# Hanbo-Cheng/DAWN-pytorch

Hardware: AMD Instinct MI355X
Metric: generated frames/sec at 256x256, 50 DDIM steps (higher is better)
Workload: dtype f32

## Files before the change

dawn-pytorch_amd/_lib.py:

```python
from __future__ import annotations

import ctypes as C
import os
from pathlib import Path

_HERE = Path(__file__).resolve().parent
LIB_PATH = Path(os.environ.get("DAWN_HIP_LIB", str(_HERE / "libdawn_hip.so")))

c_f = C.c_void_p
_i, _l, _f, _d = C.c_int, C.c_long, C.c_float, C.c_double


class ConvDesc(C.Structure):
    _fields_ = [
        ("in0", c_f), ("in1", c_f),
        ("C0", _i), ("C1", _i), ("ld0", _i), ("ld1", _i),
        ("F", _i), ("Hi", _i), ("Wi", _i), ("Ho", _i), ("Wo", _i),
        ("KH", _i), ("KW", _i), ("stride", _i), ("pad", _i),
        ("mode", _i),
        ("w", c_f), ("bias", c_f),
        ("N", _i),
        ("row_mean", c_f), ("row_rstd", c_f),
        ("ch_a", c_f), ("ch_b", c_f),
        ("pro_act", _i),
# ... 31 lines not shown
    "dawn_gn_finalize": [c_f, _d, c_f, c_f, c_f, c_f, _i, _f, c_f, c_f, c_f],
    "dawn_gn_reduce_finalize": [c_f, _i, _d, c_f, c_f, c_f, c_f, _i, _f, c_f, c_f, c_f],
    "dawn_gn_ticket_reset": [c_f, c_f],
    "dawn_gn_apply_res": [c_f, c_f, c_f, c_f, c_f, _l, _i, c_f],
    "dawn_ln_rowstats": [c_f, _i, _i, c_f, _i, _i, _l, _f, c_f, c_f, c_f],
    "dawn_ln_rows": [c_f, _i, _i, c_f, _i, _i, _l, _f, c_f, c_f],
    "dawn_xattn_prep": [c_f, _i, c_f, c_f, c_f, _i, c_f, c_f],
    "dawn_xattn_core": [c_f, c_f, _l, _i, c_f, c_f, c_f, c_f],
    "dawn_xattn_ln_sum": [c_f, c_f, c_f, _l, _i, _f, c_f],
    "dawn_xattn_tables": [c_f, c_f, c_f, c_f, c_f, c_f, _i, _i, c_f, c_f],
    "dawn_xattn_sigma_out": [c_f, _l, _i, c_f, c_f, _i, _f, c_f, c_f],
    "dawn_xattn_sigma_out_h1": [c_f, _l, _i, c_f, c_f, _i, _f, c_f, c_f, c_f, c_f, c_f],
    "dawn_xattn_layer_c64": [c_f, _i, _i, c_f, _i, _i, _l, _i, c_f, c_f, c_f, c_f, _f, c_f, c_f],
    "dawn_xattn_layer_c64_h1": [c_f, _i, _i, c_f, _i, _i, _l, _i, c_f, c_f, c_f, c_f, _f, c_f, c_f, c_f, c_f, c_f],
    "dawn_temporal_attn": [c_f, _i, _i, _i, _i, _i, c_f, c_f, c_f, c_f, c_f],
    "dawn_temporal_attn_ex": [c_f, _i, _i, _i, _i, _i, c_f, c_f, c_f, c_f, _i, c_f],
    "dawn_temporal_layer_c64": [c_f, _i, _i, _i, _i, _i, c_f, c_f, c_f, c_f, c_f, c_f, _f, c_f, c_f],
    "dawn_temporal_layer_c64_ex": [c_f, _i, _i, _i, _i, _i, c_f, c_f, c_f, c_f, c_f, c_f, c_f, _f, c_f, _i, c_f],
    "dawn_tl16_schedule": [_i, _i, _i, _i, c_f, c_f],
    "dawn_tl13_schedule": [_i, _i, _i, _i, c_f],
    "dawn_sla_context": [c_f, _i, _i, c_f, c_f],
    "dawn_sla_apply": [c_f, c_f, _i, _i, c_f, c_f],
    "dawn_sla_ws_floats": [_i, _i, _i],
    "dawn_gemm1x1_split_ok": [_l, _i, _i, _i],
    "dawn_gemm1x1_ln_inline_ok": [_l, _i, _i, _i],
    "dawn_sla_layer_c64": [c_f, _i, _i, c_f, c_f, c_f, c_f, _f, c_f, c_f, c_f],
    "dawn_frame_attn": [c_f, _i, _i, c_f, c_f],
    "dawn_init_conv_x": [c_f, c_f, c_f, _i, _i, _i, _i, c_f, c_f],
    "dawn_init_conv_x_ex": [c_f, _l, c_f, c_f, _i, _i, _i, _i, c_f, c_f],
    "dawn_head_out": [c_f, c_f, c_f, c_f, c_f, c_f, _l, _i, c_f, c_f],
    "dawn_heads_eps": [c_f, c_f, c_f, c_f, c_f, c_f, c_f, _i, _i, c_f, _i, _i, c_f, c_f, c_f, c_f, _l, _i, c_f, c_f],
    "dawn_fold_heads": [c_f, c_f, c_f, c_f, c_f, c_f, c_f, c_f, _i, _i, c_f, c_f],
    "dawn_linear": [c_f, _i, _i, _i, c_f, c_f, _i, _i, c_f, _i, c_f],
    "dawn_sinusoidal": [_f, _i, c_f, c_f, c_f],
    "dawn_ddim_x0": [c_f, c_f, _f, _f, _l, c_f, c_f, c_f],
    "dawn_select_scan": [c_f, _i, C.c_ulonglong, c_f, _i, c_f],
    "dawn_select_hist": [c_f, _l, c_f, _i, c_f, c_f],
    "dawn_select_finalize": [c_f, c_f, _f, c_f, c_f],
    "dawn_select_ws_reset": [c_f, c_f],
    "dawn_attn_bias32": [c_f, _i, c_f, _i, c_f, _i, _i, _i, _i, c_f, c_f, c_f, _i, _f, c_f, _i, c_f],
    "dawn_attn_win32": [c_f, _i, c_f, _i, c_f, _i, _i, _i, _i, _i, c_f, c_f, c_f, _i, _f, c_f, _i, c_f],
    "dawn_ubench_mfma_bf16": [_i, _i, c_f, c_f, C.POINTER(C.c_float), c_f],
    "dawn_ddim_update": [c_f, c_f, c_f, c_f, _f, _f, _f, _l, c_f, c_f],
    "dawn_cfg_combine": [c_f, c_f, _f, _l, c_f, c_f],
    "dawn_cfg_x0": [c_f, c_f, _f, c_f, _f, _f, _l, c_f, c_f, c_f, c_f],
    "dawn_workspace_bytes_guided": [c_f, _i, _i, _i, _i, _i],
# ... 97 lines not shown
CTX_SIGNATURES = {
    "dawn_ctx_create": [c_f, c_f, _i, c_f],
    "dawn_ctx_destroy": [c_f],
    "dawn_ctx_set_option": [c_f, _i, _i],
    "dawn_clip_bytes": [c_f, _i, _i, _i],
    "dawn_workspace_bytes": [c_f, _i, _i, _i],
    "dawn_workspace_bytes_sharded": [c_f, _i, _i, _i, _i, _i],
    "dawn_clip_prepare": [c_f, _i, _i, _i, c_f, c_f, _i, c_f, c_f, c_f, C.c_size_t, c_f, C.c_size_t, c_f],
    "dawn_unet_forward": _fwd + [c_f],
    "dawn_unet_forward_sharded": _fwd + [c_f, c_f],
    "dawn_sampler_run": _run + [c_f],
    "dawn_sampler_run_sharded": _run + [c_f, c_f],
    "dawn_ctx_profile_read": [c_f, c_f, _i],
    "dawn_rel_pos_bucket": [_i],
}

_lib = None


class DawnHipError(RuntimeError):
    pass


LONG_RESULT = {"dawn_sla_ws_floats", "dawn_workspace_bytes_guided", "dawn_decoder_skip_bytes", "dawn_decoder_workspace_bytes",
               "dawn_hubert_conv_frames", "dawn_hubert_workspace_bytes", "dawn_pbnet_workspace_bytes",
               "dawn_pose_blink_workspace_bytes", "dawn_clip_bytes", "dawn_workspace_bytes",
               "dawn_workspace_bytes_sharded", "dawn_image_ingest_workspace_bytes", "dawn_resample16k_len",
               "dawn_resample16k_workspace_bytes", "dawn_bundle_device_bytes",
               "dawn_bundle_verify_workspace_bytes"}


def lib() -> C.CDLL:
    global _lib
    if _lib is None:
        if not LIB_PATH.exists():
            raise DawnHipError(
                f"{LIB_PATH} not found: the HIP extension is mandatory (no CPU fallback). "
                "Build it with `python -c 'import __graft_entry__ as g; g.build()'` or ./build_lib.sh")
        L = C.CDLL(str(LIB_PATH))
        L.dawn_last_error.restype = C.c_char_p
        L.dawn_abi_version.restype = _i
        for name, args in {**SIGNATURES, **CTX_HELPER_SIGNATURES, **CTX_SIGNATURES}.items():
            fn = getattr(L, name)
            fn.argtypes = args
            fn.restype = _l if name in LONG_RESULT else _i
        _lib = L
    return _lib
# ... 6 lines not shown
```

dawn-pytorch_amd/csrc/dawn_ctx.hip:

```cpp
#include "dawn_host.h"

#include <math.h>
#include <string.h>
#include <iterator>
#include <vector>

extern "C" int dawn_gemm1x1_split_ok(long M, int N, int C0, int C1);
extern "C" int dawn_gemm1x1_ln_inline_ok(long M, int N, int C0, int C1);

namespace {

#define HCK(expr)                                                     \
    do {                                                              \
        const hipError_t e__ = (expr);                                \
        if (e__ != hipSuccess) return dawn_set_error(e__, __FILE__, __LINE__); \
    } while (0)

struct RB {
    int Cin = 0, Co = 0;
    bool conditioned = false;
    int cond_index = -1, film_off = 0;
    const float *w1 = nullptr, *b1 = nullptr, *g1 = nullptr, *be1 = nullptr, *w2 = nullptr, *b2 = nullptr, *g2 = nullptr,
                *be2 = nullptr, *wr = nullptr, *br = nullptr;
    const void *w1s = nullptr, *w2s = nullptr, *wrs = nullptr, *wqs = nullptr, *w1w = nullptr, *w2w = nullptr, *w1w4 = nullptr, *w2w4 = nullptr;
// ... 19 lines not shown
struct ProfEntry { hipEvent_t e0, e1; double flops, bytes; int kind; };

}

struct dawn_ctx {
    dawn_unet_cfg cfg;
    int dims[10];
    const float *w3, *wfea, *b_init, *sin_freqs, *t_w1, *t_b1, *t_w2, *t_b2, *film_w, *film_b, *wg, *bg, *wo, *bo;
    AT init_tattn;
    std::vector<Level> downs, ups;
    RB mid1, mid2, head_g, head_o;
    AT mid_sattn, mid_tattn;
    int n_cond = 0, film_total = 0, time_dim = 0;
    float rel_emb[32 * 8];
    float rot_freqs[16];
    const float* rot_freqs_dev = nullptr;
    std::vector<float> host_tab;
    hipStream_t side = nullptr;
    hipEvent_t ev_fork = nullptr, ev_join = nullptr;
    int conv_policy = 0, temporal_flags = 0, overlap = 1;
    int up_border = 0;
    int long_clip_frames = 4096;
    int fold_heads = 1;
    float* heads_fold = nullptr;
    Arena arena;
    bool prof_on = false;
    std::vector<ProfEntry> prof;
    std::vector<hipEvent_t> ev_pool;
};

namespace {

void load_rb(dawn_ctx* c, DawnWeights& Wt, const std::string& p, int Cin, int Co, bool conditioned, RB& rb, int& film_off) {
    auto F = [&](const std::string& n) { return Wt.getf(p + n); };
    auto V = [&](const std::string& n) { return Wt.opt(p + n); };
    rb.Cin = Cin; rb.Co = Co; rb.conditioned = conditioned;
    rb.w1 = F("w1"); rb.b1 = F("b1"); rb.g1 = F("g1"); rb.be1 = F("be1");
    rb.w2 = F("w2"); rb.b2 = F("b2"); rb.g2 = F("g2"); rb.be2 = F("be2");
    rb.w1s = V("w1s"); rb.w2s = V("w2s"); rb.w1w = V("w1w"); rb.w2w = V("w2w"); rb.w1w4 = V("w1w4"); rb.w2w4 = V("w2w4");
    if (Cin != Co) { rb.wr = F("wr"); rb.br = F("br"); rb.wrs = V("wrs"); }
    if (conditioned) {
        rb.cond_index = c->n_cond++;
        rb.film_off = film_off;
        film_off += 2 * Co;
        rb.wq = F("wq"); rb.wqs = V("wqs"); rb.q_scale = F("q_scale"); rb.g3 = F("g3");
        for (int b = 0; b < 3; ++b) {
// ... 491 lines not shown
    }
    T2 spatial_linear(const AT& a, const T2& x, int Fr, int H, int W, bool inplace = false) {
        const int HW = H * W;
        T2 o;
        if (a.C == 64) {
            float* ws = falloc((size_t)dawn_sla_ws_floats(Fr, HW, a.wqkv_s != nullptr));
            o = inplace ? x : t2(x.rows, 64);
            LAUNCH(dawn_sla_layer_c64(x.p, Fr, HW, a.wqkv, a.wqkv_s, a.wout, a.bout, 1e-5f, ws, o.p, cur));
            A.free(ws);
            return o;
        }
        return per_frame_attention(a, x, Fr, H, W, true);
    }
    T2 mid_spatial(const AT& a, const T2& x, int Fr, int H, int W) { return per_frame_attention(a, x, Fr, H, W, false); }
    T2 per_frame_attention(const AT& a, const T2& x, int Fr, int H, int W, bool linear) {
        const int HW = H * W;
        T2 o = t2(x.rows, a.C);
        const int step = Fr > c->long_clip_frames ? 256 : Fr;
        for (int fa = 0; fa < Fr; fa += step) {
            const int fb = fa + step < Fr ? fa + step : Fr, Fc = fb - fa;
            T2 xv;
            xv.p = x.p + (size_t)fa * HW * a.C; xv.rows = (long)Fc * HW; xv.C = a.C;
            T2 qkv = ln_gemm(xv, nullptr, a.wqkv, 768, a.wqkv_s, Fc, H, W);
            T2 at = t2(xv.rows, 256);
            if (linear) {
                float* ctx = falloc((size_t)Fc * 8 * 32 * 32);
                LAUNCH(dawn_sla_context(qkv.p, Fc, HW, ctx, cur));
                LAUNCH(dawn_sla_apply(qkv.p, ctx, Fc, HW, at.p, cur));
                A.free(ctx);
            } else {
                LAUNCH(dawn_frame_attn(qkv.p, Fc, HW, at.p, cur));
            }
            rel(qkv);
            ConvArgs g;
            g.in0 = at.p; g.C0 = 256; g.ld0 = 256; g.w = a.wout; g.w_bf3 = a.wout_s; g.bias = linear ? a.bout : nullptr; g.N = a.C;
            g.Fr = Fc; g.Hi = H; g.Wi = W; g.res = xv.p; g.ld_res = a.C; g.out = o.p + (size_t)fa * HW * a.C; g.ld_out = a.C;
            conv(g);
            rel(at);
        }
        return o;
    }

    void forward(const float* x3, float t, float* eps_out) {
        float* film = begin(t);
        T2 r, x;
        init_layers(x3, r, x);
// ... 266 lines not shown
    if (c->ev_join) (void)hipEventDestroy(c->ev_join);
    for (auto& p : c->prof) { (void)hipEventDestroy(p.e0); (void)hipEventDestroy(p.e1); }
    for (auto e : c->ev_pool) (void)hipEventDestroy(e);
    if (c->heads_fold) (void)hipFree(c->heads_fold);
    delete c;
}

extern "C" int dawn_ctx_set_option(dawn_ctx* c, int option, int value) {
    if (option == DAWN_OPT_UP_BORDER && (value < 0 || value > 2))
        return dawn_set_error_msg(-204, "dawn_ctx_set_option: DAWN_OPT_UP_BORDER is 0 (zero), 1 (edge) or 2 (wrap)");
    if (!c) return dawn_set_error_msg(-202, "dawn_ctx_set_option: null ctx");
    switch (option) {
        case DAWN_OPT_CONV_POLICY: c->conv_policy = value; return 0;
        case DAWN_OPT_TEMPORAL_FLAGS: c->temporal_flags = value; return 0;
        case DAWN_OPT_OVERLAP: c->overlap = value ? 1 : 0; return 0;
        case DAWN_OPT_LONG_CLIP_FRAMES: c->long_clip_frames = value > 0 ? value : 4096; return 0;
        case DAWN_OPT_UP_BORDER: c->up_border = value; return 0;
        case DAWN_OPT_FOLD_HEADS: c->fold_heads = value ? 1 : 0; return 0;
        case DAWN_OPT_PROFILE:
            c->prof_on = value != 0;
            return 0;
        default: return dawn_set_error_msg(-204, "dawn_ctx_set_option: unknown option");
    }
}

extern "C" size_t dawn_clip_bytes(dawn_ctx* c, int F, int h, int w) {
    if (!c || F <= 0 || h <= 0 || w <= 0) return 0;
    return clip_layout(c, F, h, w).total;
}

static size_t clip_scratch_bytes(dawn_ctx* c, int F, int h, int w) {
    int maxCo = 0;
    for (int l = 0; l <= c->cfg.n_levels; ++l) maxCo = c->dims[l] > maxCo ? c->dims[l] : maxCo;
    return al256((size_t)h * w * c->cfg.fea_ch * 4) + al256((size_t)F * 2 * maxCo * 4) + al256((size_t)F * 128 * 4) + 4096;
}

extern "C" int dawn_clip_prepare(dawn_ctx* c, int F, int h, int w, const float* fea272, const float* cond, int ld_cond,
                                 const float* rot_cos, const float* rot_sin, void* clip_mem, size_t clip_bytes,
                                 void* workspace, size_t workspace_bytes, void* stream) {
    if (!c || !fea272 || !cond || !clip_mem) return dawn_set_error_msg(-202, "dawn_clip_prepare: null argument");
    const ClipLayout L = clip_layout(c, F, h, w);
    if (clip_bytes < L.total) return dawn_set_error_msg(-205, "dawn_clip_prepare: clip memory too small (dawn_clip_bytes)");
    if (workspace_bytes < clip_scratch_bytes(c, F, h, w)) return dawn_set_error_msg(-201, "dawn_clip_prepare: workspace too small");
    hipStream_t s = (hipStream_t)stream;
    char* cm = (char*)clip_mem;
    char* ws = (char*)workspace;
// ... 335 lines not shown
```

dawn-pytorch_amd/csrc/spatial_attn.hip:

```cpp
#include "dawn_common.h"
#include "../../include/dawn_hip.h"

namespace {

constexpr int HEADS = 8, DH = 32, QKV = 768;

__global__ __launch_bounds__(512) void sla_context_kernel(const float* __restrict__ qkv, int HW,
                                                          float* __restrict__ ctx) {
    __shared__ float dens[HEADS * DH];
    const int f = blockIdx.x;
    const int tid = threadIdx.x;
    const int h = tid >> 6, lane = tid & 63;
    const int l31 = lane & 31, half = lane >> 5;
    const float* base = qkv + (long)f * HW * QKV + h * DH + l31;
    constexpr float LOG2E = 1.4426950408889634f;
    float kn[16], vn[16];
    auto request = [&](int t0) __attribute__((always_inline)) {
#pragma unroll
        for (int s = 0; s < 16; ++s) {
            const int n = t0 + 16 * half + s;
            const bool ok = n < HW;
            const float* r = base + (long)(ok ? n : HW - 1) * QKV;
            kn[s] = ok ? r[HEADS * DH] : -3.0e38f;
            vn[s] = ok ? r[2 * HEADS * DH] : 0.f;
// ... 79 lines not shown
            for (int c = 0; c < 4; ++c)
#pragma unroll
                for (int e = 0; e < 4; ++e) {
                    q4[c][e] = __builtin_amdgcn_exp2f((q4[c][e] - mx) * 1.4426950408889634f);
                    sm += q4[c][e];
                }
            sm += __shfl_xor(sm, 32, 64);
            const float inv = 0.17677669529663687f / sm;
            f32x16 acc;
#pragma unroll
            for (int r = 0; r < 16; ++r) acc[r] = 0.f;
#pragma unroll
            for (int c = 0; c < 4; ++c) {
                const f32x4 a4 = *reinterpret_cast<const f32x4*>(cT + (h * DH + l31) * 36 + 16 * half + 4 * c);
#pragma unroll
                for (int e = 0; e < 4; ++e) acc = __builtin_amdgcn_mfma_f32_32x32x2f32(a4[e], q4[c][e] * inv, acc, 0, 0, 0);
            }
            if (ok) {
#pragma unroll
                for (int g = 0; g < 4; ++g)
                    *reinterpret_cast<f32x4*>(orow + h * DH + 8 * g + 4 * half) =
                        f32x4{acc[4 * g], acc[4 * g + 1], acc[4 * g + 2], acc[4 * g + 3]};
            }
        }
    }
}

__global__ __launch_bounds__(64) void frame_attn_kernel(const float* __restrict__ qkv, int N,
                                                        float* __restrict__ out) {
    extern __shared__ __attribute__((aligned(16))) float kv[];
    float* ks = kv;
    float* vs = kv + (long)N * DH;
    const int f = blockIdx.x / HEADS, h = blockIdx.x % HEADS;
    const int lane = threadIdx.x;
    const float* base = qkv + (long)f * N * QKV + h * DH;
    for (int i = lane; i < N * DH; i += 64) {
        const int n = i >> 5, c = i & 31;
        ks[i] = base[(long)n * QKV + HEADS * DH + c];
        vs[i] = base[(long)n * QKV + 2 * HEADS * DH + c];
    }
    __syncthreads();
    for (int i0 = 0; i0 < N; i0 += 64) {
        const int i = i0 + lane;
        const bool ok = i < N;
        float q[DH], o[DH];
#pragma unroll
// ... 23 lines not shown
#pragma unroll
            for (int d = 0; d < DH; d += 4) {
                f32x4 v = {o[d] * inv, o[d + 1] * inv, o[d + 2] * inv, o[d + 3] * inv};
                *reinterpret_cast<f32x4*>(op + d) = v;
            }
        }
    }
}

}

extern "C" int dawn_sla_context(const float* qkv, int F, int HW, float* ctx, void* stream) {
    hipLaunchKernelGGL(sla_context_kernel, dim3(F), dim3(512), 0, (hipStream_t)stream, qkv, HW, ctx);
    DAWN_LAUNCH_CHECK();
    return 0;
}
extern "C" int dawn_sla_apply(const float* qkv, const float* ctx, int F, int HW, float* out, void* stream) {
    const int rpb = 512;
    hipLaunchKernelGGL(sla_apply_kernel, dim3(dawn_cdiv(HW, rpb), F), dim3(256), 0, (hipStream_t)stream, qkv, ctx, HW,
                       rpb, out);
    DAWN_LAUNCH_CHECK();
    return 0;
}
extern "C" int dawn_frame_attn(const float* qkv, int F, int N, float* out, void* stream) {
    if (N > 256) return dawn_set_error_msg(-40, "dawn_frame_attn: more than 256 tokens per frame not supported");
    const size_t lds = (size_t)N * DH * 2 * sizeof(float);
    hipLaunchKernelGGL(frame_attn_kernel, dim3(F * HEADS), dim3(64), lds, (hipStream_t)stream, qkv, N, out);
    DAWN_LAUNCH_CHECK();
    return 0;
}
```

dawn-pytorch_amd/ctx.py:

```python
from __future__ import annotations

import ctypes as C
import os
from typing import Dict, List, Optional, Sequence

import torch

from . import _lib
from ._lib import check
from .pack import PackedAttn, PackedResBlock, PackedUNet

Tensor = torch.Tensor


class UnetCfg(C.Structure):
    _fields_ = [("dim", C.c_int), ("n_levels", C.c_int), ("dim_mults", C.c_int * 8), ("fea_ch", C.c_int),
                ("cond_aud", C.c_int), ("cond_pose", C.c_int), ("cond_eye", C.c_int), ("win", C.c_int)]


class NamedPtr(C.Structure):
    _fields_ = [("name", C.c_char_p), ("ptr", C.c_void_p)]


class DdimStep(C.Structure):
# ... 169 lines not shown
            self._ws = None
            self._ws = torch.empty(nbytes, dtype=torch.uint8, device=self.device)
        return self._ws


class CtxEvaluator(_Evaluator):

    def __init__(self, P: PackedUNet):
        self.P = P
        cfg = UnetCfg()
        cfg.dim, cfg.n_levels = P.dim, P.n_levels
        for i in range(P.n_levels):
            cfg.dim_mults[i] = P.dims[i + 1] // P.dim
        cfg.fea_ch = P.fea_ch
        cfg.cond_aud, cfg.cond_pose, cfg.cond_eye = P.cond_dims
        cfg.win = P.win
        super().__init__("dawn_ctx_create", "dawn_ctx_destroy", cfg, named_weights(P), P.rel_emb.device, fp32_only=False)
        self._need = {}
        self._policy = 0
        if P.up_border:
            self.set_option(OPT_UP_BORDER, P.up_border)
        if os.environ.get("DAWN_FOLD_HEADS", "1") == "0":
            self.set_option(OPT_FOLD_HEADS, 0)

    def set_option(self, option: int, value: int) -> None:
        check(self.L.dawn_ctx_set_option(self.h, option, int(value)), "dawn_ctx_set_option")
        if option == OPT_CONV_POLICY:
            self._policy = int(value)
        if option != OPT_PROFILE:
            self._need.clear()

    def workspace(self, F: int, h: int, w: int, shard: Optional[ShardCallbacks] = None, guided: bool = False) -> Tensor:
        key = (F, h, w, self._policy, None if shard is None else (shard.rank, shard.world))
        if guided:
            key = key + ("guided",)
        need = self._need.get(key)
        if need is None:
            if guided:
                rank, world = (0, 1) if shard is None else (shard.rank, shard.world)
                need = self._need[key] = int(self.L.dawn_workspace_bytes_guided(self.h, F, h, w, rank, world))
            else:
                need = self._need[key] = int(self.L.dawn_workspace_bytes(self.h, F, h, w) if shard is None else
                                             self.L.dawn_workspace_bytes_sharded(self.h, F, h, w, shard.rank, shard.world))
        return self._grown(need)

    def prepare_clip(self, fea272: Tensor, cond: Tensor, rcos: Optional[Tensor] = None, rsin: Optional[Tensor] = None) -> dict:
        Cf, h, w = fea272.shape
        F = cond.shape[0]
        if not (fea272.is_cuda and fea272.is_contiguous() and cond.is_cuda and cond.stride(1) == 1 and fea272.dtype == torch.float32
                and cond.dtype == torch.float32):
            raise _lib.DawnHipError("prepare_clip: fea272 must be a contiguous fp32 GPU tensor, cond an fp32 GPU tensor with unit column stride")
        mem = torch.empty(int(self.L.dawn_clip_bytes(self.h, F, h, w)), dtype=torch.uint8, device=self.device)
        ws = self.workspace(F, h, w)
# ... 832 lines not shown
```

dawn-pytorch_amd/ops.py:

```python
from __future__ import annotations

import ctypes as C
import os
from typing import Optional, Tuple

import torch

from . import _lib
from ._lib import ConvDesc, check
from .policy import ConvPolicy

Tensor = torch.Tensor


def _p(t: Optional[Tensor]) -> Optional[int]:
    return None if t is None else t.data_ptr()


def _ld(t: Optional[Tensor]) -> int:
    return 0 if t is None else (t.stride(0) if t.dim() >= 2 else t.numel())


def _need(ok, what: str) -> None:
    if not ok:
        raise _lib.DawnHipError(f"HipOps precondition failed -- {what}")


class HipOps:

    name = "hip"

    def __init__(self, comm=None):
        self.L = _lib.lib()
        self.comm = comm
        self.prof = None
        self.prof_layers = None
        self.prof_on = True
        self.overlap = True
        self._side_stream = None
        self.graph_error = None
        self.conv_policy = 0
        self.temporal_flags = 0
        self.temporal_attn_flags = 0
        self.sk_ws = None
        self.fuse_h1 = True
        self.fold_heads = os.environ.get("DAWN_FOLD_HEADS", "1") != "0"
        self._sel_ws = {}
        self._tickets = {}
        self.fuse_gn = True

    def _gn_ticket(self, like: Tensor) -> Tensor:
        key = (like.device.index, self._stream())
        t = self._tickets.get(key)
        if t is None:
            t = self._tickets[key] = torch.empty(4, device=like.device, dtype=torch.int32)
            check(self.L.dawn_gn_ticket_reset(_p(t), self._stream()), "dawn_gn_ticket_reset")
        return t

    def begin_evaluation(self, like: Tensor) -> None:
        check(self.L.dawn_gn_ticket_reset(_p(self._gn_ticket(like)), self._stream()), "dawn_gn_ticket_reset")

    def with_comm(self, comm):
        o = HipOps(comm)
        o.prof = self.prof
        o.prof_layers = self.prof_layers
        o.prof_on = self.prof_on
        o.prof_every = getattr(self, "prof_every", 1)
        o.overlap = self.overlap
        o.conv_policy = self.conv_policy
        o.temporal_flags = self.temporal_flags
        o.temporal_attn_flags = self.temporal_attn_flags
        o.sk_ws = self.sk_ws
        o.fuse_h1 = self.fuse_h1
        o.fold_heads = self.fold_heads
        o._sel_ws = self._sel_ws
        o._tickets = self._tickets
        o.fuse_gn = self.fuse_gn
        return o

    @staticmethod
    def _require(*ts: Optional[Tensor]) -> None:
        for t in ts:
            if t is None:
                continue
            if not t.is_cuda:
                raise _lib.DawnHipError("HipOps needs GPU tensors; there is no CPU fallback on the product path")
            if t.dtype not in (torch.float32, torch.float64, torch.int32, torch.uint8) or t.stride(-1) != 1:
                raise _lib.DawnHipError(f"bad tensor for HipOps: dtype={t.dtype} strides={t.stride()}")

    @staticmethod
    def _stream() -> int:
        return torch.cuda.current_stream().cuda_stream

    def empty(self, *shape, like: Optional[Tensor] = None, dtype=torch.float32, device=None) -> Tensor:
        return torch.empty(*shape, device=like.device if like is not None else device, dtype=dtype)

    def fork_join(self, side, main):
# ... 288 lines not shown
        _need(out.is_contiguous() and out.shape == (Fq * HW, 64), "temporal_layer_c64: out.is_contiguous() and out.shape == (Fq * HW, 64)")
        ev = None
        if getattr(self, "prof_layers", None) is not None and self.prof_on:
            ev = (torch.cuda.Event(enable_timing=True), torch.cuda.Event(enable_timing=True))
            ev[0].record()
        check(self.L.dawn_temporal_layer_c64_ex(_p(x), Fext, HW, q0, Fq, win, _p(wqkv), _p(wqkv_bf3), _p(wout), _p(wout_bf3p),
                                                _p(rcos), _p(rsin), _p(band), eps, _p(out), self.temporal_flags,
                                                self._stream()),
              "dawn_temporal_layer_c64")
        if ev is not None:
            ev[1].record()
            self.prof_layers.append(("temporal_layer_c64", (Fext, HW, q0, Fq, win, wqkv_bf3 is not None and wout_bf3p is not None), ev[0], ev[1]))
        return out

    def sla(self, qkv: Tensor, F: int, HW: int) -> Tensor:
        _need(qkv.is_contiguous() and qkv.shape == (F * HW, 768), "sla: qkv.is_contiguous() and qkv.shape == (F * HW, 768)")
        ctx = self.empty(F, 8, 32, 32, like=qkv)
        out = self.empty(F * HW, 256, like=qkv)
        s = self._stream()
        check(self.L.dawn_sla_context(_p(qkv), F, HW, _p(ctx), s), "dawn_sla_context")
        check(self.L.dawn_sla_apply(_p(qkv), _p(ctx), F, HW, _p(out), s), "dawn_sla_apply")
        return out

    def sla_layer_c64(self, x: Tensor, F: int, HW: int, wqkv: Tensor, wout: Tensor, bias: Tensor,
                      eps: float = 1e-5, wqkv_bf3: Optional[Tensor] = None, out: Optional[Tensor] = None) -> Tensor:
        _need(x.is_contiguous() and x.shape == (F * HW, 64), "sla_layer_c64: x.is_contiguous() and x.shape == (F * HW, 64)")
        self._require(x, wqkv, wout, bias)
        ws = self.empty(self.L.dawn_sla_ws_floats(F, HW, int(wqkv_bf3 is not None)), like=x)
        if out is None:
            out = self.empty(F * HW, 64, like=x)
        _need(out.is_contiguous() and out.shape == (F * HW, 64), "sla_layer_c64: out.is_contiguous() and out.shape == (F * HW, 64)")
        check(self.L.dawn_sla_layer_c64(_p(x), F, HW, _p(wqkv), _p(wqkv_bf3), _p(wout), _p(bias), eps, _p(ws), _p(out),
                                        self._stream()), "dawn_sla_layer_c64")
        return out

    def frame_attn(self, qkv: Tensor, F: int, N: int) -> Tensor:
        _need(qkv.is_contiguous() and qkv.shape == (F * N, 768), "frame_attn: qkv.is_contiguous() and qkv.shape == (F * N, 768)")
        out = self.empty(F * N, 256, like=qkv)
        check(self.L.dawn_frame_attn(_p(qkv), F, N, _p(out), self._stream()), "dawn_frame_attn")
        return out

    def init_conv_x(self, x: Tensor, w3: Tensor, fea_pre: Tensor, F: int, h: int, w: int, Co: int,
                    frames: Optional[Tuple[int, int]] = None, out: Optional[Tensor] = None) -> Tensor:
        _need(x.is_contiguous() and x.shape == (3, F, h, w) and x.dtype == torch.float32, "init_conv_x: x.is_contiguous() and x.shape == (3, F, h, w) and x.dtype == torch.float32")
        self._require(x, w3, fea_pre, out)
        fa, fb = frames if frames is not None else (0, F)
# ... 561 lines not shown
```

dawn-pytorch_amd/unet_forward.py:

```python
from __future__ import annotations

from dataclasses import dataclass
from typing import List, Optional, Tuple

import torch

from .pack import PackedAttn, PackedResBlock, PackedUNet

Tensor = torch.Tensor


@dataclass
class ClipState:
    F: int
    Ttotal: int
    f0: int
    h: int
    w: int
    fea_pre: Tensor
    kvtab: List[Tensor]
    nulltab: List[Tensor]
    xtab: List[Optional[Tensor]]
    rcos: Tensor
    rsin: Tensor
# ... 240 lines not shown


def _spatial_then_temporal(ops, sp, tattn: PackedAttn, holder: list, F: int, H: int, W: int, cs: ClipState, spatial) -> Tensor:
    x = holder.pop()
    if cs.comm is None or not hasattr(cs.comm, "own_view"):
        c64 = x.shape[1] == 64
        y = spatial(ops, sp, x, F, H, W, out=x) if c64 else spatial(ops, sp, x, F, H, W)
        del x
        return _temporal(ops, tattn, y, F, H, W, cs, inplace=c64)
    HW, C = H * W, x.shape[1]

    def produce(fa, fb, o):
        spatial(ops, sp, x[fa * HW:fb * HW], fb - fa, H, W, out=o)
    own, hx = _edge_first(ops, cs, F, H, W, C, x, produce)
    del produce, x
    return _temporal(ops, tattn, own, F, H, W, cs, hx)


LONG_CLIP_FRAMES = 4096
TEMPORAL_SEG_FRAMES = 200
FRAME_CHUNK = 256


def _per_frame_attention(ops, a: PackedAttn, x: Tensor, F: int, H: int, W: int, out: Optional[Tensor], core, bias) -> Tensor:
    HW = H * W
    if F <= LONG_CLIP_FRAMES:
        qkv = _ln_gemm(ops, x, None, a.wqkv, 768, a.wqkv_s, F=F, Hi=H, Wi=W)
        o = core(qkv, F, HW)
        del qkv
        return ops.conv_gemm(o, a.wout, a.C, bias=bias, res=x, F=F, Hi=H, Wi=W, w_bf3=a.wout_s, out=out)
    if out is None:
        out = ops.empty(F * HW, a.C, like=x)
    for fa, fb in _chunks(0, F, FRAME_CHUNK):
        qkv = _ln_gemm(ops, x[fa * HW:fb * HW], None, a.wqkv, 768, a.wqkv_s, F=fb - fa, Hi=H, Wi=W)
        o = core(qkv, fb - fa, HW)
        del qkv
        ops.conv_gemm(o, a.wout, a.C, bias=bias, res=x[fa * HW:fb * HW], F=fb - fa, Hi=H, Wi=W, w_bf3=a.wout_s, out=out[fa * HW:fb * HW])
        del o
    return out


def _spatial_linear(ops, a: PackedAttn, x: Tensor, F: int, H: int, W: int, out: Optional[Tensor] = None) -> Tensor:
    if a.C == 64:
        return ops.sla_layer_c64(x, F, H * W, a.wqkv, a.wout, a.bout, wqkv_bf3=a.wqkv_s, out=out)
    return _per_frame_attention(ops, a, x, F, H, W, out, ops.sla, a.bout)


def _mid_spatial(ops, a: PackedAttn, x: Tensor, F: int, H: int, W: int, out: Optional[Tensor] = None) -> Tensor:
    return _per_frame_attention(ops, a, x, F, H, W, out, ops.frame_attn, None)


def unet_forward(ops, P: PackedUNet, cs: ClipState, x3: Tensor, t: float, film_all: Optional[Tensor] = None) -> Tensor:
    film_all = _begin(ops, P, cs, x3, t, film_all)
    return _unet_rest(ops, P, cs, x3, film_all, list(_init_layers(ops, P, cs, x3)))


def _begin(ops, P: PackedUNet, cs: ClipState, x3: Tensor, t: float, film_all: Optional[Tensor]) -> Tensor:
    if hasattr(ops, "begin_evaluation"):
        ops.begin_evaluation(x3)
    if film_all is None:
        film_all = time_film(ops, P, t, cs.fea_pre)
    if cs.comm is not None and hasattr(cs.comm, "keep_buffers"):
        cs.comm.keep_buffers = cs.F <= LONG_CLIP_FRAMES
    return film_all


def _init_layers(ops, P: PackedUNet, cs: ClipState, x3: Tensor):
    F, H, W = cs.F, cs.h, cs.w
# ... 147 lines not shown
```

include/dawn_hip.h:

```cpp
#ifndef DAWN_HIP_H
#define DAWN_HIP_H
#include <stdint.h>
#include <stddef.h>
#ifdef __cplusplus
extern "C" {
#endif

const char* dawn_last_error(void);
int dawn_abi_version(void);

typedef struct dawn_conv_desc {
    const float* in0; const float* in1;
    int C0, C1, ld0, ld1;
    int F, Hi, Wi, Ho, Wo;
    int KH, KW, stride, pad;
    int mode;
    const float* w;
    const float* bias;
    int N;
    const float* row_mean; const float* row_rstd;
    const float* ch_a; const float* ch_b;
    int pro_act;
    const float* pro_add; int ld_add;
    const float* res; int ld_res;
// ... 113 lines not shown
                          float* out, int flags, void* stream);

int dawn_temporal_layer_c64(const float* x, int Fext, int HW, int q0, int Fq, int win, const float* wqkv,
                            const void* wqkv_bf3, const float* wout, const float* rot_cos, const float* rot_sin,
                            const float* band, float eps, float* out, void* stream);
#define DAWN_TL_FORCE_MASK     7
#define DAWN_TL_FORCE_WMODE(m) ((m) + 1)
#define DAWN_TL_SCHED_HINTS    16
#define DAWN_TL_OUT_FP32       32
#define DAWN_TL_NO_FIXED200    64
#define DAWN_TL_NO_KVI         128
#define DAWN_TL_KEEP_32X32     256
int dawn_temporal_layer_c64_ex(const float* x, int Fext, int HW, int q0, int Fq, int win, const float* wqkv,
                               const void* wqkv_bf3, const float* wout, const void* wout_bf3p, const float* rot_cos,
                               const float* rot_sin, const float* band, float eps, float* out, int flags, void* stream);

typedef struct dawn_tl16_sched { unsigned w[12]; } dawn_tl16_sched;
int dawn_tl16_schedule(int Fext, int q0, int Fq, int win, dawn_tl16_sched* sched, int* simd_units);
int dawn_tl13_schedule(int Fext, int q0, int Fq, int win, unsigned* words16);

int dawn_sla_context(const float* qkv, int F, int HW, float* ctx, void* stream);
int dawn_sla_apply(const float* qkv, const float* ctx, int F, int HW, float* out, void* stream);

long dawn_sla_ws_floats(int F, int HW, int split);
int dawn_sla_layer_c64(const float* x, int F, int HW, const float* wqkv, const void* wqkv_bf3, const float* wout,
                       const float* bias, float eps, float* M_ws, float* out, void* stream);

int dawn_frame_attn(const float* qkv, int F, int N, float* out, void* stream);

int dawn_init_conv_x_ex(const float* x, long plane_stride, const float* w3, const float* fea_pre, int F, int h, int w, int Co,
                        float* out, void* stream);
int dawn_init_conv_x(const float* x, const float* w3, const float* fea_pre, int F, int h, int w, int Co,
                     float* out, void* stream);
int dawn_head_out(const float* hg, const float* ho, const float* wg, const float* bg, const float* wo,
                  const float* bo, long rows, int Co, float* eps_out, void* stream);
int dawn_heads_eps(const float* c2g, const float* a2g, const float* b2g, const float* c2o, const float* a2o, const float* b2o,
                   const float* in0, int ld0, int C0, const float* in1, int ld1, int C1, const float* wg, const float* wo,
                   const float* Wf, const float* bf, long rows, int Co, float* eps_out, void* stream);
int dawn_fold_heads(const float* wg, const float* bg, const float* wo, const float* bo, const float* wr_g, const float* br_g,
                    const float* wr_o, const float* br_o, int Co, int Cin, float* Wf, float* bf);

int dawn_linear(const float* in, int M, int K, int ld_in, const float* W, const float* bias, int N,
                int act_in, float* out, int ld_out, void* stream);
int dawn_sinusoidal(float t, int dim, const float* freqs, float* out, void* stream);

int dawn_ddim_x0(const float* x, const float* eps, float recip, float recipm1, long n, float* x0,
// ... 57 lines not shown

int dawn_attn_bias32(const float* q, int ldq, const float* k, int ldk, const float* v, int ldv, int Tq, int Tk, int heads,
                     const float* bias, const float* rot_cos, const float* rot_sin, int nrot, float scale, float* out, int ld_out,
                     void* stream);
int dawn_attn_win32(const float* q, int ldq, const float* k, int ldk, const float* v, int ldv, int Tq, int Tk, int heads, int win,
                    const float* bias_rel, const float* rot_cos, const float* rot_sin, int nrot, float scale, float* out, int ld_out,
                    void* stream);

typedef struct dawn_ctx dawn_ctx;
typedef struct dawn_unet_cfg {
    int dim;
    int n_levels;
    int dim_mults[8];
    int fea_ch;
    int cond_aud, cond_pose, cond_eye;
    int win;
} dawn_unet_cfg;
typedef struct dawn_named_ptr { const char* name; const void* ptr; } dawn_named_ptr;
int dawn_ctx_create(const dawn_unet_cfg* cfg, const dawn_named_ptr* weights, int n_weights, dawn_ctx** out);
void dawn_ctx_destroy(dawn_ctx* ctx);
enum { DAWN_OPT_CONV_POLICY = 1, DAWN_OPT_TEMPORAL_FLAGS = 2, DAWN_OPT_OVERLAP = 3, DAWN_OPT_PROFILE = 4, DAWN_OPT_LONG_CLIP_FRAMES = 5,
       DAWN_OPT_UP_BORDER = 6, DAWN_OPT_FOLD_HEADS = 7 };
int dawn_ctx_set_option(dawn_ctx* ctx, int option, int value);
size_t dawn_clip_bytes(dawn_ctx* ctx, int F, int h, int w);
size_t dawn_workspace_bytes(dawn_ctx* ctx, int F, int h, int w);
int dawn_clip_prepare(dawn_ctx* ctx, int F, int h, int w, const float* fea272, const float* cond, int ld_cond,
                      const float* rot_cos, const float* rot_sin, void* clip_mem, size_t clip_bytes, void* workspace,
                      size_t workspace_bytes, void* stream);
int dawn_unet_forward(dawn_ctx* ctx, int F, int h, int w, const void* clip_mem, const float* x3, float t,
                      float* eps_out, void* workspace, size_t workspace_bytes, void* stream);
typedef struct dawn_ddim_step {
    int t, t_next;
    float recip, recipm1;
    float sqrt_alpha_next, c, sigma;
} dawn_ddim_step;
int dawn_sampler_run(dawn_ctx* ctx, int F, int h, int w, const void* clip_mem, const float* x_init, int S,
                     const dawn_ddim_step* steps, uint64_t seed, const float* const* noises, float* x_out,
                     float* thresholds, void* workspace, size_t workspace_bytes, void* stream);
typedef struct dawn_shard_comm {
    void* user;
    int rank, world;
    int (*halo_begin)(void* user, float* xe, int hl, int F, int hh, long frame_floats, void* stream);
    int (*halo_end)(void* user, void* stream);
    int (*allreduce_sum_f64)(void* user, double* buf, int n, void* stream);
    int (*allreduce_sum_u32)(void* user, unsigned* buf, int n, void* stream);
    int (*allreduce_min_u32)(void* user, unsigned* buf, int n, void* stream);
// ... 213 lines not shown
```

Before: 181.8.

## Fold linear-attention context into output projection per frame

For linear spatial attention with C of 128, 256 or 512, each frame's per-head context matrix is pre-multiplied with the output projection weights into a small per-frame matrix (split into three bf16 parts). A new MFMA kernel then applies softmaxed queries directly against that matrix and adds bias and residual. This replaces the separate attention-apply pass and the output 1x1 GEMM, removing the intermediate 256-wide attention tensor round trip through memory. The fold costs extra work per frame, so it is gated on HW >= 2C, and the bf16 triple split adds a precision-emulation risk.

```diff
diff --git a/dawn-pytorch_amd/_lib.py b/dawn-pytorch_amd/_lib.py
--- a/dawn-pytorch_amd/_lib.py
+++ b/dawn-pytorch_amd/_lib.py
@@ -77,6 +77,10 @@
     "dawn_sla_context": [c_f, _i, _i, c_f, c_f],
     "dawn_sla_apply": [c_f, c_f, _i, _i, c_f, c_f],
     "dawn_sla_ws_floats": [_i, _i, _i],
+    "dawn_sla_out_ws_floats": [_i, _i, _i],
+    "dawn_sla_out_pays": [_i, _i],
+    "dawn_ctx_set_fold_attn_out": [c_f, _i],
+    "dawn_sla_out": [c_f, _i, _i, _i, c_f, c_f, c_f, c_f, c_f, c_f],
     "dawn_gemm1x1_split_ok": [_l, _i, _i, _i],
     "dawn_gemm1x1_ln_inline_ok": [_l, _i, _i, _i],
     "dawn_sla_layer_c64": [c_f, _i, _i, c_f, c_f, c_f, c_f, _f, c_f, c_f, c_f],
@@ -220,7 +224,7 @@
     pass
 
 
-LONG_RESULT = {"dawn_sla_ws_floats", "dawn_workspace_bytes_guided", "dawn_decoder_skip_bytes", "dawn_decoder_workspace_bytes",
+LONG_RESULT = {"dawn_sla_ws_floats", "dawn_sla_out_ws_floats", "dawn_workspace_bytes_guided", "dawn_decoder_skip_bytes", "dawn_decoder_workspace_bytes",
                "dawn_hubert_conv_frames", "dawn_hubert_workspace_bytes", "dawn_pbnet_workspace_bytes",
                "dawn_pose_blink_workspace_bytes", "dawn_clip_bytes", "dawn_workspace_bytes",
                "dawn_workspace_bytes_sharded", "dawn_image_ingest_workspace_bytes", "dawn_resample16k_len",
diff --git a/dawn-pytorch_amd/csrc/dawn_ctx.hip b/dawn-pytorch_amd/csrc/dawn_ctx.hip
--- a/dawn-pytorch_amd/csrc/dawn_ctx.hip
+++ b/dawn-pytorch_amd/csrc/dawn_ctx.hip
@@ -65,6 +65,7 @@
     int up_border = 0;
     int long_clip_frames = 4096;
     int fold_heads = 1;
+    int fold_attn_out = 1;
     float* heads_fold = nullptr;
     Arena arena;
     bool prof_on = false;
@@ -602,6 +603,14 @@
             T2 xv;
             xv.p = x.p + (size_t)fa * HW * a.C; xv.rows = (long)Fc * HW; xv.C = a.C;
             T2 qkv = ln_gemm(xv, nullptr, a.wqkv, 768, a.wqkv_s, Fc, H, W);
+            const long fold_ws = linear && c->fold_attn_out && step == Fr && dawn_sla_out_pays(HW, a.C) ? dawn_sla_out_ws_floats(Fc, HW, a.C) : 0;
+            if (fold_ws) {
+                float* ws = falloc((size_t)fold_ws);
+                LAUNCH(dawn_sla_out(qkv.p, Fc, HW, a.C, a.wout, a.bout, xv.p, ws, o.p + (size_t)fa * HW * a.C, cur));
+                A.free(ws);
+                rel(qkv);
+                continue;
+            }
             T2 at = t2(xv.rows, 256);
             if (linear) {
                 float* ctx = falloc((size_t)Fc * 8 * 32 * 32);
@@ -914,6 +923,12 @@
             return 0;
         default: return dawn_set_error_msg(-204, "dawn_ctx_set_option: unknown option");
     }
+}
+
+extern "C" int dawn_ctx_set_fold_attn_out(dawn_ctx* c, int on) {
+    if (!c) return dawn_set_error_msg(-202, "dawn_ctx_set_fold_attn_out: null ctx");
+    c->fold_attn_out = on ? 1 : 0;
+    return 0;
 }
 
 extern "C" size_t dawn_clip_bytes(dawn_ctx* c, int F, int h, int w) {
diff --git a/dawn-pytorch_amd/csrc/spatial_attn.hip b/dawn-pytorch_amd/csrc/spatial_attn.hip
--- a/dawn-pytorch_amd/csrc/spatial_attn.hip
+++ b/dawn-pytorch_amd/csrc/spatial_attn.hip
@@ -125,6 +125,160 @@
                     *reinterpret_cast<f32x4*>(orow + h * DH + 8 * g + 4 * half) =
                         f32x4{acc[4 * g], acc[4 * g + 1], acc[4 * g + 2], acc[4 * g + 3]};
             }
+        }
+    }
+}
+
+constexpr int FOLD_FLOATS_PER_FRAME_AND_CHANNEL = HEADS * 2 * 3 * 2 * 16 / 4;
+
+__global__ __launch_bounds__(256) void sla_fold_kernel(const float* __restrict__ ctx, const float* __restrict__ wout, int C,
+                                                       unsigned char* __restrict__ Mp) {
+    __shared__ float cs[DH * DH];
+    const int h = blockIdx.x, f = blockIdx.y, tid = threadIdx.x;
+    const float* ch = ctx + ((long)f * HEADS + h) * DH * DH;
+    for (int i = tid; i < DH * DH; i += 256) cs[i] = ch[i];
+    __syncthreads();
+    for (int u = tid; u < 4 * C; u += 256) {
+        const int n = u % C, hf = (u / C) & 1, j = u / (2 * C);
+        const float* cr = cs + (16 * hf + 8 * j) * DH;
+        float m8[8];
+#pragma unroll
+        for (int i = 0; i < 8; ++i) m8[i] = 0.f;
+#pragma unroll
+        for (int e4 = 0; e4 < 8; ++e4) {
+            const f32x4 w4 = *reinterpret_cast<const f32x4*>(wout + ((size_t)(h * 8 + e4) * C + n) * 4);
+#pragma unroll
+            for (int s = 0; s < 4; ++s)
+#pragma unroll
+                for (int i = 0; i < 8; ++i) m8[i] = __builtin_fmaf(cr[i * DH + 4 * e4 + s], w4[s], m8[i]);
+        }
+        bf16x8 p0, p1, p2;
+        dawn_split3_oct(m8, p0, p1, p2);
+        unsigned char* dst = Mp + ((((size_t)f * HEADS + h) * 2 + j) * 6 + hf) * C * 16 + (size_t)n * 16;
+        *reinterpret_cast<bf16x8*>(dst) = p0;
+        *reinterpret_cast<bf16x8*>(dst + (size_t)2 * C * 16) = p1;
+        *reinterpret_cast<bf16x8*>(dst + (size_t)4 * C * 16) = p2;
+    }
+}
+
+template <int NCH>
+__global__ __launch_bounds__(256) void sla_out_apply_kernel(const float* __restrict__ qkv, const unsigned char* __restrict__ Mp,
+                                                            const float* __restrict__ bias, const float* x, int HW, int C, float* out) {
+    constexpr int CC = 128 * NCH, TPB = 4 / NCH, NV = 6 * CC / 256;
+    constexpr int NB = NCH == 1 ? 4 : 3, AHEAD = NB - 1, NU = 2 * HEADS;
+    __shared__ __attribute__((aligned(16))) unsigned char As[NB][6 * CC * 16];
+    const int f = blockIdx.y, c0 = blockIdx.z * CC;
+    const int tid = threadIdx.x;
+    const int wave = tid >> 6, lane = tid & 63;
+    const int l31 = lane & 31, half = lane >> 5;
+    const int cw = c0 + 128 * (wave % NCH);
+    const int ntiles = HW >> 5, tile = blockIdx.x * TPB + wave / NCH;
+    const bool active = tile < ntiles;
+    const long row = (long)f * HW + 32 * (active ? tile : ntiles - 1) + l31;
+    const float* qr = qkv + row * QKV + 16 * half;
+    const unsigned char* mf = Mp + (size_t)f * 16 * 6 * C * 16 + (size_t)c0 * 16;
+
+    const int wv = __builtin_amdgcn_readfirstlane(wave);
+    const unsigned char* src[NV];
+#pragma unroll
+    for (int v = 0; v < NV; ++v) {
+        const int i = tid + 256 * v;
+        src[v] = mf + ((size_t)(i / CC) * C + i % CC) * 16;
+    }
+    const size_t unit_bytes = (size_t)6 * C * 16;
+    auto fetch = [&](int un, int buf) __attribute__((always_inline)) {
+#pragma unroll
+        for (int v = 0; v < NV; ++v)
+            __builtin_amdgcn_global_load_lds((const __attribute__((address_space(1))) void*)(src[v] + (size_t)un * unit_bytes),
+                                             (__attribute__((address_space(3))) void*)(As[buf] + (wv * 64 + 256 * v) * 16), 16, 0, 0);
+    };
+    f32x4 qn[4];
+    auto request_q = [&](int h) __attribute__((always_inline)) {
+#pragma unroll
+        for (int c = 0; c < 4; ++c) qn[c] = *reinterpret_cast<const f32x4*>(qr + h * DH + 4 * c);
+    };
+#pragma unroll
+    for (int u = 0; u < AHEAD; ++u) fetch(u, u);
+    request_q(0);
+    asm volatile("s_waitcnt vmcnt(0)" ::: "memory");
+    __syncthreads();
+    int buf = 0;
+    f32x16 acc[4];
+#pragma unroll
+    for (int nt = 0; nt < 4; ++nt) acc[nt] = zero16();
+#pragma unroll 1
+    for (int h = 0; h < HEADS; ++h) {
+        f32x4 q4[4];
+#pragma unroll
+        for (int c = 0; c < 4; ++c) q4[c] = qn[c];
+        float mx = fmaxf(fmaxf(q4[0].x, q4[0].y), fmaxf(q4[0].z, q4[0].w));
+#pragma unroll
+        for (int c = 1; c < 4; ++c) mx = fmaxf(mx, fmaxf(fmaxf(q4[c].x, q4[c].y), fmaxf(q4[c].z, q4[c].w)));
+        mx = fmaxf(mx, __shfl_xor(mx, 32, 64));
+        float sm = 0.f;
+#pragma unroll
+        for (int c = 0; c < 4; ++c)
+#pragma unroll
+            for (int e = 0; e < 4; ++e) {
+                q4[c][e] = __builtin_amdgcn_exp2f((q4[c][e] - mx) * 1.4426950408889634f);
+                sm += q4[c][e];
+            }
+        sm += __shfl_xor(sm, 32, 64);
+        const float inv = 0.17677669529663687f / sm;
+        bf16x8 qb[2][3];
+#pragma unroll
+        for (int j = 0; j < 2; ++j) {
+            float q8[8];
+#pragma unroll
+            for (int i = 0; i < 8; ++i) q8[i] = q4[2 * j + (i >> 2)][i & 3] * inv;
+            dawn_split3_oct(q8, qb[j][0], qb[j][1], qb[j][2]);
+        }
+        request_q(h + 1 < HEADS ? h + 1 : h);
+#pragma unroll
+        for (int j = 0; j < 2; ++j) {
+            const int un = 2 * h + j;
+            __builtin_amdgcn_sched_barrier(0);
+            fetch(un + AHEAD < NU ? un + AHEAD : NU - 1, buf == 0 ? NB - 1 : buf - 1);
+            bf16x8 a[4][3];
+#pragma unroll
+            for (int nt = 0; nt < 4; ++nt)
+#pragma unroll
+                for (int pl = 0; pl < 3; ++pl)
+                    a[nt][pl] = *reinterpret_cast<const bf16x8*>(As[buf] + ((size_t)((pl * 2 + half) * CC + (cw - c0) + 32 * nt + l31)) * 16);
+            __builtin_amdgcn_sched_barrier(0);
+#pragma unroll
+            for (int nt = 0; nt < 4; ++nt)
+#pragma unroll
+                for (int u = 0; u < 6; ++u)
+                    acc[nt] = __builtin_amdgcn_mfma_f32_32x32x16_bf16(a[nt][DAWN_SPLIT6_A[u]], qb[j][DAWN_SPLIT6_B[u]], acc[nt], 0, 0, 0);
+            const float sink = (acc[0][15] + acc[1][15]) + (acc[2][15] + acc[3][15]);
+            asm volatile("" :: "v"(sink));
+            __builtin_amdgcn_sched_barrier(0);
+            asm volatile("s_waitcnt vmcnt(%0)" ::"n"((AHEAD - 1) * NV) : "memory");
+            __builtin_amdgcn_s_barrier();
+            buf = buf + 1 == NB ? 0 : buf + 1;
+        }
+    }
+    asm volatile("s_waitcnt vmcnt(0)" ::: "memory");
+    if (active) {
+        const float* xrow = x + row * C;
+        float* orow = out + row * C;
+#pragma unroll
+        for (int np = 0; np < 4; np += 2) {
+            f32x4 xres[2][4];
+#pragma unroll
+            for (int nt = 0; nt < 2; ++nt)
+#pragma unroll
+                for (int g = 0; g < 4; ++g) xres[nt][g] = *reinterpret_cast<const f32x4*>(xrow + cw + 32 * (np + nt) + 8 * g + 4 * half);
+#pragma unroll
+            for (int nt = 0; nt < 2; ++nt)
+#pragma unroll
+                for (int g = 0; g < 4; ++g) {
+                    const int ch = cw + 32 * (np + nt) + 8 * g + 4 * half;
+                    const f32x4 b4 = *reinterpret_cast<const f32x4*>(bias + ch);
+                    const f32x4 o = {acc[np + nt][4 * g], acc[np + nt][4 * g + 1], acc[np + nt][4 * g + 2], acc[np + nt][4 * g + 3]};
+                    *reinterpret_cast<f32x4*>(orow + ch) = o + b4 + xres[nt][g];
+                }
         }
     }
 }
@@ -194,6 +348,28 @@
     DAWN_LAUNCH_CHECK();
     return 0;
 }
+extern "C" long dawn_sla_out_ws_floats(int F, int HW, int C) {
+    if (F <= 0 || F > 65535 || HW <= 0 || HW % 32 != 0 || (C != 128 && C != 256 && C != 512)) return 0;
+    return (long)F * (HEADS * DH * DH + FOLD_FLOATS_PER_FRAME_AND_CHANNEL * C);
+}
+extern "C" int dawn_sla_out_pays(int HW, int C) { return HW >= 2 * C; }
+extern "C" int dawn_sla_out(const float* qkv, int F, int HW, int C, const float* wout, const float* bias, const float* x, float* ws,
+                            float* out, void* stream) {
+    if (dawn_sla_out_ws_floats(F, HW, C) == 0) return 1;
+    if (!qkv || !wout || !bias || !x || !ws || !out) return dawn_set_error_msg(-41, "dawn_sla_out: null argument");
+    hipStream_t s = (hipStream_t)stream;
+    float* ctx = ws;
+    unsigned char* Mp = reinterpret_cast<unsigned char*>(ws + (size_t)F * HEADS * DH * DH);
+    hipLaunchKernelGGL(sla_context_kernel, dim3(F), dim3(512), 0, s, qkv, HW, ctx);
+    DAWN_LAUNCH_CHECK();
+    hipLaunchKernelGGL(sla_fold_kernel, dim3(HEADS, F), dim3(256), 0, s, ctx, wout, C, Mp);
+    DAWN_LAUNCH_CHECK();
+    const int ntiles = HW / 32;
+    if (C == 128) hipLaunchKernelGGL(sla_out_apply_kernel<1>, dim3(dawn_cdiv(ntiles, 4), F, 1), dim3(256), 0, s, qkv, Mp, bias, x, HW, C, out);
+    else hipLaunchKernelGGL(sla_out_apply_kernel<2>, dim3(dawn_cdiv(ntiles, 2), F, C / 256), dim3(256), 0, s, qkv, Mp, bias, x, HW, C, out);
+    DAWN_LAUNCH_CHECK();
+    return 0;
+}
 extern "C" int dawn_frame_attn(const float* qkv, int F, int N, float* out, void* stream) {
     if (N > 256) return dawn_set_error_msg(-40, "dawn_frame_attn: more than 256 tokens per frame not supported");
     const size_t lds = (size_t)N * DH * 2 * sizeof(float);
diff --git a/dawn-pytorch_amd/ctx.py b/dawn-pytorch_amd/ctx.py
--- a/dawn-pytorch_amd/ctx.py
+++ b/dawn-pytorch_amd/ctx.py
@@ -215,6 +215,8 @@
             self.set_option(OPT_UP_BORDER, P.up_border)
         if os.environ.get("DAWN_FOLD_HEADS", "1") == "0":
             self.set_option(OPT_FOLD_HEADS, 0)
+        if os.environ.get("DAWN_FOLD_ATTN_OUT", "1") == "0":
+            self.set_fold_attn_out(False)
 
     def set_option(self, option: int, value: int) -> None:
         check(self.L.dawn_ctx_set_option(self.h, option, int(value)), "dawn_ctx_set_option")
@@ -222,6 +224,10 @@
             self._policy = int(value)
         if option != OPT_PROFILE:
             self._need.clear()
+
+    def set_fold_attn_out(self, on: bool) -> None:
+        check(self.L.dawn_ctx_set_fold_attn_out(self.h, int(bool(on))), "dawn_ctx_set_fold_attn_out")
+        self._need.clear()
 
     def workspace(self, F: int, h: int, w: int, shard: Optional[ShardCallbacks] = None, guided: bool = False) -> Tensor:
         key = (F, h, w, self._policy, None if shard is None else (shard.rank, shard.world))
diff --git a/dawn-pytorch_amd/ops.py b/dawn-pytorch_amd/ops.py
--- a/dawn-pytorch_amd/ops.py
+++ b/dawn-pytorch_amd/ops.py
@@ -45,6 +45,7 @@
         self.sk_ws = None
         self.fuse_h1 = True
         self.fold_heads = os.environ.get("DAWN_FOLD_HEADS", "1") != "0"
+        self.fold_attn_out = os.environ.get("DAWN_FOLD_ATTN_OUT", "1") != "0"
         self._sel_ws = {}
         self._tickets = {}
         self.fuse_gn = True
@@ -73,6 +74,7 @@
         o.sk_ws = self.sk_ws
         o.fuse_h1 = self.fuse_h1
         o.fold_heads = self.fold_heads
+        o.fold_attn_out = self.fold_attn_out
         o._sel_ws = self._sel_ws
         o._tickets = self._tickets
         o.fuse_gn = self.fuse_gn
@@ -407,6 +409,25 @@
         check(self.L.dawn_sla_apply(_p(qkv), _p(ctx), F, HW, _p(out), s), "dawn_sla_apply")
         return out
 
+    def sla_out_pays(self, HW: int, C: int) -> bool:
+        return bool(self.L.dawn_sla_out_pays(HW, C))
+
+    def sla_out(self, qkv: Tensor, F: int, HW: int, x: Tensor, wout: Tensor, bias: Tensor, out: Optional[Tensor] = None) -> Optional[Tensor]:
+        C = x.shape[1]
+        _need(qkv.is_contiguous() and qkv.shape == (F * HW, 768) and x.is_contiguous() and x.shape == (F * HW, C),
+              "sla_out: qkv contiguous (F * HW, 768), x contiguous (F * HW, C)")
+        n = self.L.dawn_sla_out_ws_floats(F, HW, C)
+        if n == 0:
+            return None
+        _need(wout.is_contiguous() and wout.numel() == 256 * C and bias is not None and bias.numel() == C, "sla_out: wout (64, C, 4), bias (C,)")
+        self._require(qkv, x, wout, bias, out)
+        ws = self.empty(n, like=qkv)
+        if out is None:
+            out = self.empty(F * HW, C, like=x)
+        _need(out.is_contiguous() and out.shape == (F * HW, C), "sla_out: out.is_contiguous() and out.shape == (F * HW, C)")
+        check(self.L.dawn_sla_out(_p(qkv), F, HW, C, _p(wout), _p(bias), _p(x), _p(ws), _p(out), self._stream()), "dawn_sla_out")
+        return out
+
     def sla_layer_c64(self, x: Tensor, F: int, HW: int, wqkv: Tensor, wout: Tensor, bias: Tensor,
                       eps: float = 1e-5, wqkv_bf3: Optional[Tensor] = None, out: Optional[Tensor] = None) -> Tensor:
         _need(x.is_contiguous() and x.shape == (F * HW, 64), "sla_layer_c64: x.is_contiguous() and x.shape == (F * HW, 64)")
diff --git a/dawn-pytorch_amd/unet_forward.py b/dawn-pytorch_amd/unet_forward.py
--- a/dawn-pytorch_amd/unet_forward.py
+++ b/dawn-pytorch_amd/unet_forward.py
@@ -286,10 +286,14 @@
 FRAME_CHUNK = 256
 
 
-def _per_frame_attention(ops, a: PackedAttn, x: Tensor, F: int, H: int, W: int, out: Optional[Tensor], core, bias) -> Tensor:
+def _per_frame_attention(ops, a: PackedAttn, x: Tensor, F: int, H: int, W: int, out: Optional[Tensor], core, bias, core_out=None) -> Tensor:
     HW = H * W
     if F <= LONG_CLIP_FRAMES:
         qkv = _ln_gemm(ops, x, None, a.wqkv, 768, a.wqkv_s, F=F, Hi=H, Wi=W)
+        if core_out is not None and hasattr(ops, core_out) and getattr(ops, "fold_attn_out", True) and getattr(ops, core_out + "_pays")(HW, a.C):
+            y = getattr(ops, core_out)(qkv, F, HW, x, a.wout, bias, out=out)
+            if y is not None:
+                return y
         o = core(qkv, F, HW)
         del qkv
         return ops.conv_gemm(o, a.wout, a.C, bias=bias, res=x, F=F, Hi=H, Wi=W, w_bf3=a.wout_s, out=out)
@@ -307,7 +311,7 @@
 def _spatial_linear(ops, a: PackedAttn, x: Tensor, F: int, H: int, W: int, out: Optional[Tensor] = None) -> Tensor:
     if a.C == 64:
         return ops.sla_layer_c64(x, F, H * W, a.wqkv, a.wout, a.bout, wqkv_bf3=a.wqkv_s, out=out)
-    return _per_frame_attention(ops, a, x, F, H, W, out, ops.sla, a.bout)
+    return _per_frame_attention(ops, a, x, F, H, W, out, ops.sla, a.bout, core_out="sla_out")
 
 
 def _mid_spatial(ops, a: PackedAttn, x: Tensor, F: int, H: int, W: int, out: Optional[Tensor] = None) -> Tensor:
diff --git a/include/dawn_hip.h b/include/dawn_hip.h
--- a/include/dawn_hip.h
+++ b/include/dawn_hip.h
@@ -159,6 +159,11 @@
 int dawn_sla_context(const float* qkv, int F, int HW, float* ctx, void* stream);
 int dawn_sla_apply(const float* qkv, const float* ctx, int F, int HW, float* out, void* stream);
 
+long dawn_sla_out_ws_floats(int F, int HW, int C);
+int dawn_sla_out_pays(int HW, int C);
+int dawn_sla_out(const float* qkv, int F, int HW, int C, const float* wout, const float* bias, const float* x, float* ws, float* out,
+                 void* stream);
+
 long dawn_sla_ws_floats(int F, int HW, int split);
 int dawn_sla_layer_c64(const float* x, int F, int HW, const float* wqkv, const void* wqkv_bf3, const float* wout,
                        const float* bias, float eps, float* M_ws, float* out, void* stream);
@@ -262,6 +267,7 @@
 enum { DAWN_OPT_CONV_POLICY = 1, DAWN_OPT_TEMPORAL_FLAGS = 2, DAWN_OPT_OVERLAP = 3, DAWN_OPT_PROFILE = 4, DAWN_OPT_LONG_CLIP_FRAMES = 5,
        DAWN_OPT_UP_BORDER = 6, DAWN_OPT_FOLD_HEADS = 7 };
 int dawn_ctx_set_option(dawn_ctx* ctx, int option, int value);
+int dawn_ctx_set_fold_attn_out(dawn_ctx* ctx, int on);
 size_t dawn_clip_bytes(dawn_ctx* ctx, int F, int h, int w);
 size_t dawn_workspace_bytes(dawn_ctx* ctx, int F, int h, int w);
 int dawn_clip_prepare(dawn_ctx* ctx, int F, int h, int w, const float* fea272, const float* cond, int ld_cond,
```

Result: no change. 182.1 (median of 5 runs) (+0.2%).
